# gnovack/distributed-training-and-deepspeed

Measured on AMD Instinct MI355X. Metric: tokens/sec (whole node) BERT-base DDP, higher is better.
Workload: dtype bf16; 1 GPU; model=bert-base-cased, params=108340804, global_batch=1024, per_gpu_batch=1024, seq_len=512, parallelism=dp1, grad_dtype=bfloat16, impl=fused, mlm_head=sparse (labelled rows only, static capacity 80896; identical loss/grads), optimizer=fused AdamW (transformers.AdamW hyper-params, lr 5e-5), tuned_gemms=True, hip_graph=False, force_collectives=False, prewarm=auto, async_wgrad=False, opt_overlap=True

## Files before the change

distributed_training_and_deepspeed_amd/ops/csrc/attention.hip:

```cpp
#include <stdio.h>
#include <type_traits>
#include <stdlib.h>
#include <string.h>

#include "common.h"

#ifndef DTD_ATTN_FUSED_BWD
#define DTD_ATTN_FUSED_BWD 0
#endif

using namespace dtd;

typedef float f32x16 __attribute__((ext_vector_type(16)));

namespace {

constexpr float kLog2e = 1.4426950408889634f;
constexpr float kLn2 = 0.6931471805599453f;

typedef short s16x4 __attribute__((ext_vector_type(4)));
typedef __attribute__((address_space(3))) s16x4 lds_s16x4;

__device__ __forceinline__ f32x16 mfma32(bf16x8 a, bf16x8 b, f32x16 c) {
  return __builtin_amdgcn_mfma_f32_32x32x16_bf16(a, b, c, 0, 0, 0);
// ... 396 lines not shown
    const bool slow = needmask || sl2 != 0.f;
    float tmax = -INFINITY;
    scores_kb(Knext, nxt, 0);
    if (slow) {
#pragma unroll
      for (int kb = 0; kb < NKB; ++kb)
#pragma unroll
        for (int i = 0; i < 16; ++i) {
          const int key = k0 + kb * 32 + crow(i, hh);
          float sv = fmaf(cur[kb][i], sc2, sl2 * (float)key);
          if (needmask && (key >= S || (a.causal && key > q))) sv = -INFINITY;
          cur[kb][i] = sv;
          tmax = fmaxf(tmax, sv);
        }
    } else {
#pragma unroll
      for (int kb = 0; kb < NKB; ++kb)
#pragma unroll
        for (int i = 0; i < 16; ++i) tmax = fmaxf(tmax, cur[kb][i]);
      tmax *= sc2;
    }
    tmax = xhalf_max(tmax);
    if (!__all(tmax - m <= a.thr)) {
      const float mnew = fmaxf(m, tmax);
      const float alpha = m == -INFINITY ? 0.f : fexp2(m - mnew);
      m = mnew;
      l *= alpha;
#pragma unroll
      for (int d = 0; d < NDB; ++d) oacc[d] *= alpha;
    }
    scores_kb(Knext, nxt, 1);
    const float mexp = m == -INFINITY ? 0.f : m;
    const float msc = slow ? 1.f : sc2;
    float ps[4];
#pragma unroll
    for (int kb = 0; kb < NKB; ++kb)
#pragma unroll
      for (int i = 0; i < 16; ++i) {
        const float pv = fexp2(fmaf(cur[kb][i], msc, -mexp));
        ps[i & 3] = (kb == 0 && i < 4) ? pv : ps[i & 3] + pv;
        cur[kb][i] = pv;
      }
    l += (ps[0] + ps[1]) + (ps[2] + ps[3]);
    if (drop) {
#pragma unroll
      for (int kb = 0; kb < NKB; ++kb) {
        const uint32_t mw = half_word(mwc[kb], hh);
#pragma unroll
        for (int i = 0; i < 16; ++i) cur[kb][i] = keep_bits(cur[kb][i], mw, crow(i, 0));
      }
    }
#pragma unroll
    for (int kb = 0; kb < NKB; ++kb)
#pragma unroll
      for (int s2 = 0; s2 < 2; ++s2) {
        bf16x8 pf;
#pragma unroll
        for (int j = 0; j < 8; ++j) pf[j] = (bf16)cur[kb][8 * s2 + j];
#pragma unroll
        for (int d = 0; d < NDB; ++d) oacc[d] = mfma32(tr_operand(V, VP, kb * 32 + 16 * s2, d * 32, lane), pf, oacc[d]);
      }
    if (t + 1 < nt) {
      if (t + 2 < nt) kl.store(Ks[t & 1], KP);
      vl.store(Vs[(t + 1) & 1], VP);
#pragma unroll
      for (int j = 0; j < NKB; ++j) mwc[j] = mwn[j];
      kl.load(ksrc, min(t + 3, last) * BN);
      vl.load(vsrc, min(t + 2, last) * BN);
      load_words(min(t + 2, last) * BN, mwn);
    }
    __syncthreads();
  };
  f32x16 sA[NKB], sB[NKB];
#pragma unroll
  for (int kb = 0; kb < NKB; ++kb) scores_kb(Ks[0], sA, kb);
  for (int t = 0; t < nt; t += 2) {
    tile_step(sA, sB, Ks[1], t);
    if (t + 1 < nt) tile_step(sB, sA, Ks[0], t + 1);
  }
  l = xhalf_sum(l);
  if (!qvalid) return;
  const float inv_l = l > 0.f ? inv_keep / l : 0.f;
  bf16* op = a.o + (size_t)(b * S + q) * a.ldo + h * D;
#pragma unroll
  for (int d = 0; d < NDB; ++d)
#pragma unroll
    for (int gq = 0; gq < 4; ++gq) {
      bf16x4 v4;
#pragma unroll
      for (int t = 0; t < 4; ++t) v4[t] = (bf16)(oacc[d][4 * gq + t] * inv_l);
      *reinterpret_cast<bf16x4*>(op + d * 32 + 8 * gq + 4 * hh) = v4;
    }
  if (hh == 0) a.lse[(size_t)bh * S + q] = (m + log2f(l)) * kLn2;
}

struct BwdArgs {
  const bf16* q; const bf16* k; const bf16* v; const bf16* dout; const float* lse; float* delta;
  const bf16* o;
  bf16* dq; bf16* dk; bf16* dv; const float* slopes;
  const uint32_t* maskA; const uint32_t* maskB;
  int B, S, H, ld, ldo, causal, W;
  float scale, p;
  float* bias_part;
  const int* kv_range;
  __device__ __forceinline__ int hkv() const { return W; }
  __device__ __forceinline__ int window() const { return __float_as_int(p); }
  __device__ __forceinline__ const int* doc() const { return kv_range; }
};

template <int S_>
__device__ __forceinline__ float xswz(float x) {
  return __int_as_float(__builtin_amdgcn_ds_swizzle(__float_as_int(x), (S_ << 10) | 0x1f));
}
template <int S_, int N>
__device__ __forceinline__ void rs_step(const float (&in)[2 * N], float (&out)[N], int r) {
  const bool hi = (r & S_) != 0;
#pragma unroll
  for (int j = 0; j < N; ++j) {
    const float mine = hi ? in[j + N] : in[j];
    const float other = hi ? in[j] : in[j + N];
    out[j] = mine + xswz<S_>(other);
  }
}
__device__ __forceinline__ float colsum32(const float (&v)[32], int r) {
  float a16[16], a8[8], a4[4], a2[2], a1[1];
  rs_step<16, 16>(v, a16, r);
  rs_step<8, 8>(a16, a8, r);
  rs_step<4, 4>(a8, a4, r);
  rs_step<2, 2>(a4, a2, r);
  rs_step<1, 1>(a2, a1, r);
  return a1[0];
}
__device__ __forceinline__ int colsum_col(int k, int hh) { return (k >> 4) * 32 + crow(k & 15, hh); }

template <int D, int OCC, int BM, bool DROP, bool ALIBI, bool MASK = true, bool RANGE = false>
__global__ void __launch_bounds__(256, OCC) attn_bwd_dkdv_kernel(BwdArgs a) {
  constexpr bool DOC = false, GQA = false, WIN = false;
#include "attention_bwd_dkdv_body.h"
}
template <int D, int OCC, int BM, bool DROP, bool ALIBI>
__global__ void __launch_bounds__(256, OCC) attn_bwd_dkdv_doc_kernel(BwdArgs a) {
  constexpr bool MASK = true, RANGE = false, DOC = true, GQA = false, WIN = false;
#include "attention_bwd_dkdv_body.h"
}
template <int D, int OCC, int BM, int MODE>
__global__ void __launch_bounds__(256, OCC) attn_bwd_dkdv_gqa_kernel(BwdArgs a) {
  constexpr bool DROP = false, ALIBI = false, MASK = true, RANGE = MODE == 1, DOC = MODE == 2, GQA = true, WIN = false;
#include "attention_bwd_dkdv_body.h"
}
template <int D, int OCC, int BM, int MODE>
__global__ void __launch_bounds__(256, OCC) attn_bwd_dkdv_win_kernel(BwdArgs a) {
  constexpr bool DROP = false, ALIBI = false, MASK = true, RANGE = MODE == 1, DOC = MODE == 2, GQA = true, WIN = true;
#include "attention_bwd_dkdv_body.h"
}

template <int D, int OCC, int BN, int RING, bool PK = false, bool RANGE = false>
__global__ void __launch_bounds__(256, OCC) attn_bwd_dq_kernel(BwdArgs a) {
  constexpr bool DOC = false, GQA = false, WIN = false;
#include "attention_bwd_dq_body.h"
}
template <int D, int OCC, int BN, int RING>
__global__ void __launch_bounds__(256, OCC) attn_bwd_dq_doc_kernel(BwdArgs a) {
  constexpr bool PK = false, RANGE = false, DOC = true, GQA = false, WIN = false;
#include "attention_bwd_dq_body.h"
}
template <int D, int OCC, int BN, int RING, int MODE>
__global__ void __launch_bounds__(256, OCC) attn_bwd_dq_gqa_kernel(BwdArgs a) {
  constexpr bool PK = false, RANGE = MODE == 1, DOC = MODE == 2, GQA = true, WIN = false;
#include "attention_bwd_dq_body.h"
}
template <int D, int OCC, int BN, int RING, int MODE>
__global__ void __launch_bounds__(256, OCC) attn_bwd_dq_win_kernel(BwdArgs a) {
  constexpr bool PK = false, RANGE = MODE == 1, DOC = MODE == 2, GQA = true, WIN = true;
#include "attention_bwd_dq_body.h"
}

#if DTD_ATTN_FUSED_BWD
__device__ __forceinline__ f32x4 mfma16(bf16x8 a, bf16x8 b, f32x4 c) {
  return __builtin_amdgcn_mfma_f32_16x16x32_bf16(a, b, c, 0, 0, 0);
}

__device__ __forceinline__ void mfma32_a(f32x16& acc, bf16x8 a, bf16x8 b) {
  asm volatile("s_nop 1\n\tv_mfma_f32_32x32x16_bf16 %0, %1, %2, %0" : "+a"(acc) : "v"(a), "v"(b));
}

__device__ __forceinline__ void mfma32_v0(f32x16& acc, bf16x8 a, bf16x8 b) {
  asm volatile("s_nop 1\n\tv_mfma_f32_32x32x16_bf16 %0, %1, %2, 0" : "=&v"(acc) : "v"(a), "v"(b));
}
__device__ __forceinline__ void mfma32_v(f32x16& acc, bf16x8 a, bf16x8 b) {
  asm volatile("s_nop 1\n\tv_mfma_f32_32x32x16_bf16 %0, %1, %2, %0" : "+v"(acc) : "v"(a), "v"(b));
}
__device__ __forceinline__ void mfma_vgpr_wait(f32x16& x, f32x16& y) {
  asm volatile("s_nop 11" : "+v"(x), "+v"(y));
}
__device__ __forceinline__ void mfma16_v(f32x4& acc, bf16x8 a, bf16x8 b) {
  asm volatile("s_nop 1\n\tv_mfma_f32_16x16x32_bf16 %0, %1, %2, %0" : "+v"(acc) : "v"(a), "v"(b));
}

template <int NKB, bool DROP>
__global__ void __launch_bounds__(256, 1) attn_bwd_fused_kernel(BwdArgs a) {
  constexpr int D = 64, NC = 4, NDB = 2, SK = 128 * NKB, KPW = 32 * NKB, NT = SK / 32;
  constexpr int KH = NKB % 2 == 0 ? 2 : 1, NH = NKB / KH;
  constexpr int DSP = 36;
  constexpr int DSR = 4 * KH * 32;
  struct Smem {
    float lse_s[32], del_s[32];
    bf16 Qs[32 * 64];
    bf16 Os[32 * 64];
    bf16 DS[DSR * DSP];
    bf16 Ks[SK * 64];
    bf16 Vs[SK * 64];
  };
  __shared__ __attribute__((aligned(16))) Smem sm;

  const int tid = threadIdx.x, lane = tid & 63, w = __builtin_amdgcn_readfirstlane(tid >> 6), hh = lane >> 5,
            r = lane & 31;
  const int bh = blockIdx.x, b = bh / a.H, h = bh % a.H;
  const int S = a.S;
  const float sc2 = a.scale * kLog2e;
  const float inv_keep = DROP ? 1.f / (1.f - a.p) : 1.f;
  const int kw0 = w * KPW;
  const int Sp = 32 * a.W;
  const float* lseb = a.lse + (size_t)bh * S;
  const RowSrc qsrc = row_src<D>(a.q + (size_t)b * S * a.ld + h * D, a.ld, S);
  const RowSrc dsrc = row_src<D>(a.dout + (size_t)b * S * a.ldo + h * D, a.ldo, S);
  const RowSrc osrc = row_src<D>(a.o + (size_t)b * S * a.ldo + h * D, a.ldo, S);
  {
    const RowSrc ksrc = row_src<D>(a.k + (size_t)b * S * a.ld + h * D, a.ld, S);
    const RowSrc vsrc = row_src<D>(a.v + (size_t)b * S * a.ld + h * D, a.ld, S);
#pragma unroll
    for (int half = 0; half < 2; ++half) {
      TileLoader<D, SK / 2> kl, vl;
      kl.load(ksrc, half * (SK / 2));
      vl.load(vsrc, half * (SK / 2));
      kl.store_swz(sm.Ks + half * (SK / 2) * 64);
      vl.store_swz(sm.Vs + half * (SK / 2) * 64);
    }
  }
  TileLoader<D, 32> ql, dl, ol;
  float lse_n = 0.f;
  auto fetch = [&](int q0) {
    ql.load(qsrc, q0);
    dl.load(dsrc, q0);
    ol.load(osrc, q0);
    if (tid < 32) lse_n = lseb[q0 + tid];
  };
  auto stage = [&]() {
    float part = 0.f;
#pragma unroll
    for (int j = 0; j < 8; ++j) part = fmaf((float)dl.reg[0][j], (float)ol.reg[0][j], part);
    part += __shfl_xor(part, 1, 64);
    part += __shfl_xor(part, 2, 64);
    part += __shfl_xor(part, 4, 64);
    ql.store_swz(sm.Qs);
    dl.store_swz(sm.Os);
    if ((tid & 7) == 0) sm.del_s[tid >> 3] = -part;
    if (tid < 32) sm.lse_s[tid] = -lse_n * kLog2e;
  };
  fetch(0);
  stage();

  f32x16 dk[NKB][NDB], dv[NKB][NDB];
#pragma unroll
  for (int kb = 0; kb < NKB; ++kb)
#pragma unroll
    for (int d = 0; d < NDB; ++d) { dk[kb][d] = f32x16{}; dv[kb][d] = f32x16{}; }
  const int g16 = lane >> 4, l16 = lane & 15, qq = l16 >> 2, pp = l16 & 3;
  const int kcol = 16 * w + 4 * pp;
  __syncthreads();

  for (int t = 0; t < NT; ++t) {
    const int q0 = t * 32;
    if (t + 1 < NT) fetch(q0 + 32);
    f32x4 dq2[2] = {f32x4{}, f32x4{}};
#pragma unroll
    for (int hf = 0; hf < NH; ++hf) {
#pragma unroll
      for (int kk = 0; kk < KH; ++kk) {
        const int kb = hf * KH + kk;
        const int key0 = kw0 + 32 * kb;
        f32x16 sacc, pacc;
#pragma unroll
        for (int c = 0; c < NC; ++c) {
          const bf16x8 qa = swz_row_read(sm.Qs, 0, r, 2 * c + hh), kr = swz_row_read(sm.Ks, key0, r, 2 * c + hh);
          const bf16x8 oa = swz_row_read(sm.Os, 0, r, 2 * c + hh), vr = swz_row_read(sm.Vs, key0, r, 2 * c + hh);
          if (c == 0) { mfma32_v0(sacc, qa, kr); mfma32_v0(pacc, oa, vr); }
          else { mfma32_v(sacc, qa, kr); mfma32_v(pacc, oa, vr); }
        }
        mfma_vgpr_wait(sacc, pacc);
        uint64_t mk[16];
        if constexpr (DROP) {
          const cu64* mp = (const cu64*)(uintptr_t)(a.maskA + ((size_t)bh * a.W + min(w * NKB + kb, a.W - 1)) * Sp +
                                                    keep_off(q0, Sp));
#pragma unroll
          for (int i = 0; i < 16; ++i) mk[i] = mp[i];
        }
        f32x4 L4[4];
#pragma unroll
        for (int g = 0; g < 4; ++g) L4[g] = *reinterpret_cast<const f32x4*>(&sm.lse_s[8 * g + 4 * hh]);
        const f32x2 sc2v = pk2(sc2, sc2);
#pragma unroll
        for (int i = 0; i < 16; i += 2) {
          const f32x2 x = pk_fma(pk2(sacc[i], sacc[i + 1]), sc2v, pk2(L4[i >> 2][i & 3], L4[i >> 2][(i & 3) + 1]));
          sacc[i] = fexp2(x.x);
          sacc[i + 1] = fexp2(x.y);
        }
// ... 229 lines not shown
      for (int g = 0; g < 4; ++g) L4[g] = *reinterpret_cast<const f32x4*>(&sm.lse_s[8 * g + 4 * hh]);
      const f32x2 sc2v = pk2(sc2, sc2);
#pragma unroll
      for (int i = 0; i < 16; i += 2) {
        const f32x2 x = pk_fma(pk2(sacc[i], sacc[i + 1]), sc2v, pk2(L4[i >> 2][i & 3], L4[i >> 2][(i & 3) + 1]));
        sacc[i] = fexp2(x.x);
        sacc[i + 1] = fexp2(x.y);
      }
      f32x4 D4[4];
#pragma unroll
      for (int g = 0; g < 4; ++g) D4[g] = *reinterpret_cast<const f32x4*>(&sm.del_s[8 * g + 4 * hh]);
#pragma unroll
      for (int i = 0; i < 16; i += 2) {
        const f32x2 nd = pk2(D4[i >> 2][i & 3], D4[i >> 2][(i & 3) + 1]);
        if constexpr (DROP) {
          const f32x2 tt = pk_fma(pk2(sel_keep(pacc[i], mk[i]), sel_keep(pacc[i + 1], mk[i + 1])),
                                  pk2(inv_keep, inv_keep), nd);
          const f32x2 ds = pk2(sacc[i], sacc[i + 1]) * tt;
          pacc[i] = ds.x;
          pacc[i + 1] = ds.y;
          sacc[i] = sel_keep(sacc[i], mk[i]);
          sacc[i + 1] = sel_keep(sacc[i + 1], mk[i + 1]);
        } else {
          const f32x2 ds = pk2(sacc[i], sacc[i + 1]) * (pk2(pacc[i], pacc[i + 1]) + nd);
          pacc[i] = ds.x;
          pacc[i + 1] = ds.y;
        }
      }
      bf16* dsrow = sm.DS + (w * 32 + r) * DSP + 4 * hh;
#pragma unroll
      for (int s2 = 0; s2 < 2; ++s2) {
        bf16x8 pb, sb;
#pragma unroll
        for (int j = 0; j < 8; ++j) { pb[j] = (bf16)sacc[8 * s2 + j]; sb[j] = (bf16)pacc[8 * s2 + j]; }
#pragma unroll
        for (int d = 0; d < NDB; ++d) {
          dv[kb][d] = mfma32(tr_operand_swz(sm.Os, 16 * s2, d * 32, lane), pb, dv[kb][d]);
          dk[kb][d] = mfma32(tr_operand_swz(sm.Qs, 16 * s2, d * 32, lane), sb, dk[kb][d]);
        }
        *reinterpret_cast<bf16x4*>(dsrow + 16 * s2) = __builtin_shufflevector(sb, sb, 0, 1, 2, 3);
        *reinterpret_cast<bf16x4*>(dsrow + 16 * s2 + 8) = __builtin_shufflevector(sb, sb, 4, 5, 6, 7);
      }
      __syncthreads();
#pragma unroll 1
      for (int k0 = 0; k0 < DSR; k0 += 32) {
        const int key = (k0 / 32) * KPW + kb * 32 + 8 * g16 + qq;
        const bf16* ka = sm.Ks + key * 64 + 8 * ((kcol >> 3) ^ swz64(key)) + (kcol & 7);
        const bf16* kb4 = sm.Ks + (key + 4) * 64 + 8 * ((kcol >> 3) ^ swz64(key + 4)) + (kcol & 7);
        const int lr = k0 + 8 * g16 + qq;
        const bf16* dp = sm.DS + lr * DSP + 16 * qh + 4 * pp;
        dq1 = mfma16(cat(tr_read(ka), tr_read(kb4)), cat(tr_read(dp), tr_read(dp + 4 * DSP)), dq1);
      }
      float cs[4] = {0.f, 0.f, 0.f, 0.f};
      if (kb == NH - 1) {
        bf16x4 v4;
#pragma unroll
        for (int j = 0; j < 4; ++j) {
          v4[j] = (bf16)(dq1[j] * a.scale);
          cs[j] = (float)v4[j];
        }
        *reinterpret_cast<bf16x4*>(a.dq + (size_t)(b * S + q0 + 16 * qh + l16) * a.ld + h * D + 16 * dd + 4 * g16) = v4;
        if (a.bias_part) {
#pragma unroll
          for (int j = 0; j < 4; ++j) {
            cs[j] += __shfl_xor(cs[j], 1, 64);
            cs[j] += __shfl_xor(cs[j], 2, 64);
            cs[j] += __shfl_xor(cs[j], 4, 64);
            cs[j] += __shfl_xor(cs[j], 8, 64);
          }
          if (qh == 1 && l16 == 0)
            *reinterpret_cast<f32x4*>(&sm.csq[16 * dd + 4 * g16]) = f32x4{cs[0], cs[1], cs[2], cs[3]};
        }
        if (t + 1 < NT) stage();
      }
      __syncthreads();
      if (kb == NH - 1 && a.bias_part && qh == 0 && l16 == 0) {
        const f32x4 o4 = *reinterpret_cast<const f32x4*>(&sm.csq[16 * dd + 4 * g16]);
        *reinterpret_cast<f32x4*>(a.bias_part + ((size_t)b * (S / 32) + t) * (3 * a.H * D) + h * D + 16 * dd + 4 * g16) =
            f32x4{cs[0] + o4[0], cs[1] + o4[1], cs[2] + o4[2], cs[3] + o4[3]};
      }
    }
  }
  const float dv_scale = inv_keep;
  auto put = [&](const f32x16 (&acc)[NDB], float sc, bf16* dst, int colbase, int kb) {
    if (a.bias_part) {
      float vk[32];
#pragma unroll
      for (int d = 0; d < NDB; ++d)
#pragma unroll
        for (int i = 0; i < 16; ++i) vk[16 * d + i] = (float)(bf16)(acc[d][i] * sc);
      const float sk = colsum32(vk, r);
      a.bias_part[((size_t)b * (S / 32) + w * NKBW + kb) * (3 * a.H * D) + colbase + h * D + colsum_col(r, hh)] = sk;
    }
    bf16* p = dst + (size_t)(b * S + kw0 + 32 * kb + r) * a.ld + h * D;
#pragma unroll
    for (int d = 0; d < NDB; ++d)
#pragma unroll
      for (int gq = 0; gq < 4; ++gq) {
        bf16x4 k4;
#pragma unroll
        for (int j = 0; j < 4; ++j) k4[j] = (bf16)(acc[d][4 * gq + j] * sc);
        *reinterpret_cast<bf16x4*>(p + d * 32 + 8 * gq + 4 * hh) = k4;
      }
  };
#pragma unroll
  for (int kb = 0; kb < NKBW; ++kb) {
    put(dk[kb], a.scale, a.dk, a.H * D, kb);
    __builtin_amdgcn_sched_barrier(0);
    put(dv[kb], dv_scale, a.dv, 2 * a.H * D, kb);
    __builtin_amdgcn_sched_barrier(0);
  }
}

#endif

}

static int occupancy(int which) {
  static const int defaults[3] = {3, 2, 3};
  const char* env = getenv("DTD_ATTN_OCC");
  if (!env) return defaults[which];
  int v[3] = {defaults[0], defaults[1], defaults[2]};
  sscanf(env, "%d,%d,%d", &v[0], &v[1], &v[2]);
  return v[which];
}

static bool fwd_pipe() {
  const char* e = getenv("DTD_ATTN_FWD");
  return e != nullptr && strcmp(e, "pipe") == 0;
}

static bool fwd_pk() {
  const char* e = getenv("DTD_ATTN_FWD_PK");
  return e != nullptr && e[0] == '1';
}

static int tile_keys(int which) {
  static const int defaults[2] = {64, 64};
  const char* env = getenv("DTD_ATTN_TILE");
  if (!env) return defaults[which];
  int v[2] = {defaults[0], defaults[1]};
  sscanf(env, "%d,%d", &v[0], &v[1]);
  return v[which];
}

static int g_bwd_form = -1;
static int bwd_form() {
  if (g_bwd_form < 0) {
    const char* e = getenv("DTD_ATTN_BWD");
    g_bwd_form = !e ? 0 : strcmp(e, "fused") == 0 ? 1 : strcmp(e, "fused4") == 0 ? 2 : 0;
  }
  return g_bwd_form;
}
static bool bwd_fused() { return bwd_form() != 0; }
static bool bwd_fused8() { return bwd_form() == 1; }


enum Family { kMha = 0, kGqa = 1, kWin = 2 };

static int mode_of(const int* kv_range, const int* doc) { return doc ? 2 : kv_range ? 1 : 0; }

template <int N, class F>
static void with_const(int v, F&& f) {
  if (v >= N - 1) return f(std::integral_constant<int, N - 1>{});
  if constexpr (N > 1) with_const<N - 1>(v, f);
}
template <class F>
static void with_family(Family fam, F&& f) {
  if (fam == kMha) f(std::integral_constant<int, kMha>{});
  else if (fam == kGqa) f(std::integral_constant<int, kGqa>{});
  else f(std::integral_constant<int, kWin>{});
}

static bool offsets_fit(int S, int ld, int ldo) {
  const long long lim = 0x7fffffffLL;
  const long long W = (S + 31) / 32;
  return (long long)S * ld * 2 < lim && (long long)S * ldo * 2 < lim && 32 * W * W * 4 < lim;
}

static int check_call(Family fam, int B, int S, int H, int Hkv, int D, int ld, int ldo, int causal, int window,
                      const int* kv_range, const int* doc) {
  if (B * S * H == 0) return -1;
  if (fam == kWin && (window <= 0 || !causal)) return (int)hipErrorInvalidValue;
  if (fam != kMha && (Hkv <= 0 || Hkv > H || H % Hkv || (fam == kGqa && Hkv == H))) return (int)hipErrorInvalidValue;
  if (kv_range && doc) return (int)hipErrorInvalidValue;
  if (D != 64 && D != 128) return (int)hipErrorInvalidValue;
  if (!offsets_fit(S, ld, ldo)) return (int)hipErrorInvalidValue;
  return 0;
}

static float rescale_thr() {
  const char* e = getenv("DTD_ATTN_RESCALE_THR");
  return e ? (float)atof(e) : kRescaleThr;
}

static float window_bits(int window) {
  float f;
  memcpy(&f, &window, sizeof f);
  return f;
}

static FwdArgs fwd_args(const void* q, const void* k, const void* v, void* o, float* lse, const float* slopes,
                        const uint32_t* masks, int B, int S, int H, int ld, int ldo, int causal, float scale, float p,
                        int hkv, int window, const int* kv_range, const int* doc) {
  const int W = (S + 31) / 32;
  FwdArgs a{(const bf16*)q, (const bf16*)k, (const bf16*)v, (bf16*)o, lse, slopes, masks,
            masks ? masks + (size_t)B * H * (32 * W) * W : nullptr, B, S, H, ld, ldo, causal, hkv ? hkv : W,
            scale, p, rescale_thr(), doc ? doc : kv_range};
  if (window) a.causal = 1, a.p = window_bits(window < S ? window : S);
  return a;
}
static BwdArgs bwd_args(const void* q, const void* k, const void* v, const void* o, const void* dout, const float* lse,
                        float* delta, const uint32_t* masks, void* dq, void* dk, void* dv, const float* slopes, int B,
                        int S, int H, int ld, int ldo, int causal, float scale, float p, float* bias_part, int hkv,
                        int window, const int* kv_range, const int* doc) {
  const int W = (S + 31) / 32;
  BwdArgs a{(const bf16*)q, (const bf16*)k, (const bf16*)v, (const bf16*)dout, lse, delta, (const bf16*)o,
            (bf16*)dq, (bf16*)dk, (bf16*)dv, slopes, masks, masks ? masks + (size_t)B * H * (32 * W) * W : nullptr,
            B, S, H, ld, ldo, causal, hkv ? hkv : W, scale, p, bias_part, doc ? doc : kv_range};
  if (window) a.causal = 1, a.p = window_bits(window < S ? window : S);
  return a;
}

template <int D> struct TileForm;
template <> struct TileForm<64> { static constexpr int OCC = 3, BN = 64, RING = 1, KV_OCC = 2, KV_BM = 128; };
template <> struct TileForm<128> { static constexpr int OCC = 1, BN = 64, RING = 2, KV_OCC = 1, KV_BM = 64; };

static void launch_masks(uint32_t* masks, int B, int S, int H, float p, const uint64_t* rng, uint32_t sid, hipStream_t s) {
  const int W = (S + 31) / 32;
  hipLaunchKernelGGL(attn_mask_kernel, dim3((S + 255) / 256, B * H), dim3(256), 0, s, masks,
                     masks + (size_t)B * H * (32 * W) * W, S, W, rng, sid, keep_threshold(p));
}

template <int D>
static void launch_fwd_plain(dim3 grid, hipStream_t s, const FwdArgs& a) {
  if constexpr (D == 128) {
    hipLaunchKernelGGL((attn_fwd_kernel<128, 1, 64, 2>), grid, dim3(256), 0, s, a);
  } else if (fwd_pipe()) {
    hipLaunchKernelGGL((attn_fwd_pipe_kernel<64, 2, 64>), grid, dim3(256), 0, s, a);
  } else {
    const int o = occupancy(0);
    if (o >= 3 && fwd_pk()) hipLaunchKernelGGL((attn_fwd_kernel<64, 3, 64, 1, true>), grid, dim3(256), 0, s, a);
    else if (o >= 3) hipLaunchKernelGGL((attn_fwd_kernel<64, 3, 64, 1>), grid, dim3(256), 0, s, a);
    else if (o == 2) hipLaunchKernelGGL((attn_fwd_kernel<64, 2, 64, 2>), grid, dim3(256), 0, s, a);
    else hipLaunchKernelGGL((attn_fwd_kernel<64, 1, 64, 2>), grid, dim3(256), 0, s, a);
  }
}

template <int D, int FAM, int MODE>
static void launch_fwd_form(dim3 grid, hipStream_t s, const FwdArgs& a) {
  using T = TileForm<D>;
  if constexpr (FAM == kWin) hipLaunchKernelGGL((attn_fwd_win_kernel<D, T::OCC, T::BN, T::RING, MODE>), grid, dim3(256), 0, s, a);
  else if constexpr (FAM == kGqa) hipLaunchKernelGGL((attn_fwd_gqa_kernel<D, T::OCC, T::BN, T::RING, MODE>), grid, dim3(256), 0, s, a);
  else if constexpr (MODE == 2) hipLaunchKernelGGL((attn_fwd_doc_kernel<D, T::OCC, T::BN, T::RING>), grid, dim3(256), 0, s, a);
  else if constexpr (MODE == 1) hipLaunchKernelGGL((attn_fwd_kernel<D, T::OCC, T::BN, T::RING, false, true>), grid, dim3(256), 0, s, a);
  else launch_fwd_plain<D>(grid, s, a);
}

static int attn_fwd_launch(Family fam, const void* q, const void* k, const void* v, void* o, float* lse,
                           const float* slopes, uint32_t* masks, int B, int S, int H, int Hkv, int D, int ld, int ldo,
                           int causal, float scale, float p, const uint64_t* rng, uint32_t sid, int window,
                           const int* kv_range, const int* doc, hipStream_t s) {
  if (const int rc = check_call(fam, B, S, H, Hkv, D, ld, ldo, causal, window, kv_range, doc)) return rc < 0 ? 0 : rc;
  if (p > 0.f && !masks) return (int)hipErrorInvalidValue;
  if (p > 0.f && rng) launch_masks(masks, B, S, H, p, rng, sid, s);
  const FwdArgs a = fwd_args(q, k, v, o, lse, slopes, p > 0.f ? masks : nullptr, B, S, H, ld, ldo, causal, scale, p,
                             fam == kMha ? 0 : Hkv, window, kv_range, doc);
  const dim3 grid((S + 127) / 128, B * H);
  with_family(fam, [&](auto f) { with_const<3>(mode_of(kv_range, doc), [&](auto m) {
    constexpr int FAM = decltype(f)::value, MODE = decltype(m)::value;
    if (D == 64) launch_fwd_form<64, FAM, MODE>(grid, s, a);
    else launch_fwd_form<128, FAM, MODE>(grid, s, a);
  }); });
  DTD_LAUNCH_CHECK();
}

DTD_EXPORT int dtd_attn_fwd(const void* q, const void* k, const void* v, void* o, float* lse, const float* slopes,
                            uint32_t* masks, int B, int S, int H, int D, int ld, int ldo, int causal, float scale,
                            float p, const uint64_t* rng, uint32_t sid, hipStream_t s) {
  return attn_fwd_launch(kMha, q, k, v, o, lse, slopes, masks, B, S, H, H, D, ld, ldo, causal, scale, p, rng, sid, 0,
                         nullptr, nullptr, s);
}

DTD_EXPORT int dtd_attn_fwd_range(const void* q, const void* k, const void* v, void* o, float* lse,
                                  const float* slopes, uint32_t* masks, int B, int S, int H, int D, int ld, int ldo,
                                  int causal, float scale, float p, const uint64_t* rng, uint32_t sid,
                                  const int* kv_range, hipStream_t s) {
  if (!kv_range) return (int)hipErrorInvalidValue;
  return attn_fwd_launch(kMha, q, k, v, o, lse, slopes, masks, B, S, H, H, D, ld, ldo, causal, scale, p, rng, sid, 0,
                         kv_range, nullptr, s);
}

DTD_EXPORT int dtd_attn_fwd_doc(const void* q, const void* k, const void* v, void* o, float* lse, const float* slopes,
                                uint32_t* masks, int B, int S, int H, int D, int ld, int ldo, int causal, float scale,
                                float p, const uint64_t* rng, uint32_t sid, const int* doc, hipStream_t s) {
  if (!doc) return (int)hipErrorInvalidValue;
  return attn_fwd_launch(kMha, q, k, v, o, lse, slopes, masks, B, S, H, H, D, ld, ldo, causal, scale, p, rng, sid, 0,
                         nullptr, doc, s);
}

DTD_EXPORT int dtd_attn_fwd_gqa(const void* q, const void* k, const void* v, void* o, float* lse, int B, int S, int H,
                                int Hkv, int D, int ld, int ldo, int causal, float scale, const int* kv_range,
                                const int* doc, hipStream_t s) {
  return attn_fwd_launch(kGqa, q, k, v, o, lse, nullptr, nullptr, B, S, H, Hkv, D, ld, ldo, causal, scale, 0.f, nullptr,
                         0, 0, kv_range, doc, s);
}

DTD_EXPORT int dtd_attn_fwd_win(const void* q, const void* k, const void* v, void* o, float* lse, int B, int S, int H,
                                int Hkv, int D, int ld, int ldo, int causal, float scale, int window,
                                const int* kv_range, const int* doc, hipStream_t s) {
  return attn_fwd_launch(kWin, q, k, v, o, lse, nullptr, nullptr, B, S, H, Hkv, D, ld, ldo, causal, scale, 0.f, nullptr,
                         0, window, kv_range, doc, s);
}

DTD_EXPORT int dtd_attn_fused_bwd_built() { return DTD_ATTN_FUSED_BWD; }

DTD_EXPORT int dtd_attn_set_bwd_form(int f) {
  const int old = bwd_form();
  g_bwd_form = f < 0 || f > 2 ? 0 : f;
  return old;
}

DTD_EXPORT int dtd_attn_masks(uint32_t* masks, int B, int S, int H, float p, const uint64_t* rng, uint32_t sid,
                              hipStream_t s) {
  if (B * S * H == 0 || p <= 0.f) return 0;
  if (!masks || !rng) return (int)hipErrorInvalidValue;
  launch_masks(masks, B, S, H, p, rng, sid, s);
  DTD_LAUNCH_CHECK();
}

template <int D, int OCC, int BM>
static void launch_dkdv(dim3 grid, hipStream_t s, const BwdArgs& a) {
  const bool drop = a.maskB != nullptr, alibi = a.slopes != nullptr;
  if (!a.causal && a.S % 128 == 0 && !alibi) {
    if (drop) hipLaunchKernelGGL((attn_bwd_dkdv_kernel<D, OCC, BM, true, false, false>), grid, dim3(256), 0, s, a);
    else hipLaunchKernelGGL((attn_bwd_dkdv_kernel<D, OCC, BM, false, false, false>), grid, dim3(256), 0, s, a);
    return;
  }
  if (drop && alibi) hipLaunchKernelGGL((attn_bwd_dkdv_kernel<D, OCC, BM, true, true>), grid, dim3(256), 0, s, a);
  else if (drop) hipLaunchKernelGGL((attn_bwd_dkdv_kernel<D, OCC, BM, true, false>), grid, dim3(256), 0, s, a);
  else if (alibi) hipLaunchKernelGGL((attn_bwd_dkdv_kernel<D, OCC, BM, false, true>), grid, dim3(256), 0, s, a);
  else hipLaunchKernelGGL((attn_bwd_dkdv_kernel<D, OCC, BM, false, false>), grid, dim3(256), 0, s, a);
}

template <int D, int OCC, int BM, int MODE>
static void launch_dkdv_masked(dim3 grid, hipStream_t s, const BwdArgs& a) {
  with_const<2>(a.maskB != nullptr, [&](auto drop) { with_const<2>(a.slopes != nullptr, [&](auto alibi) {
    constexpr bool DROP = decltype(drop)::value, ALIBI = decltype(alibi)::value;
    if constexpr (MODE == 2) hipLaunchKernelGGL((attn_bwd_dkdv_doc_kernel<D, OCC, BM, DROP, ALIBI>), grid, dim3(256), 0, s, a);
    else hipLaunchKernelGGL((attn_bwd_dkdv_kernel<D, OCC, BM, DROP, ALIBI, true, true>), grid, dim3(256), 0, s, a);
  }); });
}

static int g_bwd_kernels = 3;
DTD_EXPORT int dtd_attn_set_bwd_kernels(int mask) {
  const int old = g_bwd_kernels;
  g_bwd_kernels = mask & 3;
  return old;
}

template <int D>
static void launch_bwd_plain(dim3 grid, bool run_dq, bool run_dkdv, hipStream_t s, const BwdArgs& a) {
#if DTD_ATTN_FUSED_BWD
  if (D == 64 && !a.causal && !a.slopes && a.S % 128 == 0 && a.S <= 512 && bwd_fused()) {
    const bool drop = a.maskA != nullptr;
    const dim3 g1(a.B * a.H);
    if (a.S == 512 && bwd_fused8()) {
      if (drop) hipLaunchKernelGGL((attn_bwd_fused8_kernel<2, true>), g1, dim3(512), 0, s, a);
      else hipLaunchKernelGGL((attn_bwd_fused8_kernel<2, false>), g1, dim3(512), 0, s, a);
      return;
    }
    switch (a.S / 128) {
      case 1: if (drop) hipLaunchKernelGGL((attn_bwd_fused_kernel<1, true>), g1, dim3(256), 0, s, a);
              else hipLaunchKernelGGL((attn_bwd_fused_kernel<1, false>), g1, dim3(256), 0, s, a); break;
      case 2: if (drop) hipLaunchKernelGGL((attn_bwd_fused_kernel<2, true>), g1, dim3(256), 0, s, a);
              else hipLaunchKernelGGL((attn_bwd_fused_kernel<2, false>), g1, dim3(256), 0, s, a); break;
      case 3: if (drop) hipLaunchKernelGGL((attn_bwd_fused_kernel<3, true>), g1, dim3(256), 0, s, a);
              else hipLaunchKernelGGL((attn_bwd_fused_kernel<3, false>), g1, dim3(256), 0, s, a); break;
      default: if (drop) hipLaunchKernelGGL((attn_bwd_fused_kernel<4, true>), g1, dim3(256), 0, s, a);
               else hipLaunchKernelGGL((attn_bwd_fused_kernel<4, false>), g1, dim3(256), 0, s, a); break;
    }
    return;
  }
#endif
  if constexpr (D == 64) {
    const int o = occupancy(2);
    if (!run_dq) {}
    else if (tile_keys(1) == 128) hipLaunchKernelGGL((attn_bwd_dq_kernel<64, 2, 128, 2>), grid, dim3(256), 0, s, a);
    else if (o >= 3 && fwd_pk()) hipLaunchKernelGGL((attn_bwd_dq_kernel<64, 3, 64, 1, true>), grid, dim3(256), 0, s, a);
    else if (o >= 3) hipLaunchKernelGGL((attn_bwd_dq_kernel<64, 3, 64, 1>), grid, dim3(256), 0, s, a);
    else if (o == 2) hipLaunchKernelGGL((attn_bwd_dq_kernel<64, 2, 64, 2>), grid, dim3(256), 0, s, a);
    else hipLaunchKernelGGL((attn_bwd_dq_kernel<64, 1, 64, 2>), grid, dim3(256), 0, s, a);
    const int bm = getenv("DTD_ATTN_DKDV_BM") ? atoi(getenv("DTD_ATTN_DKDV_BM")) : 128;
    if (!run_dkdv) {}
    else if (bm == 128 && occupancy(1) == 1) launch_dkdv<64, 1, 128>(grid, s, a);
    else if (bm == 128) launch_dkdv<64, 2, 128>(grid, s, a);
    else if (occupancy(1) >= 2) launch_dkdv<64, 2, 64>(grid, s, a);
    else launch_dkdv<64, 1, 64>(grid, s, a);
  } else {
    if (run_dq) hipLaunchKernelGGL((attn_bwd_dq_kernel<128, 1, 64, 2>), grid, dim3(256), 0, s, a);
    if (run_dkdv) launch_dkdv<128, 1, 64>(grid, s, a);
  }
}

template <int D, int FAM, int MODE>
static void launch_bwd_form(dim3 gq, dim3 gkv, bool run_dq, bool run_dkdv, hipStream_t s, const BwdArgs& a) {
  using T = TileForm<D>;
  if constexpr (FAM == kMha && MODE == 0) return launch_bwd_plain<D>(gq, run_dq, run_dkdv, s, a);
  if (run_dq) {
    if constexpr (FAM == kWin) hipLaunchKernelGGL((attn_bwd_dq_win_kernel<D, T::OCC, T::BN, T::RING, MODE>), gq, dim3(256), 0, s, a);
    else if constexpr (FAM == kGqa) hipLaunchKernelGGL((attn_bwd_dq_gqa_kernel<D, T::OCC, T::BN, T::RING, MODE>), gq, dim3(256), 0, s, a);
    else if constexpr (MODE == 2) hipLaunchKernelGGL((attn_bwd_dq_doc_kernel<D, T::OCC, T::BN, T::RING>), gq, dim3(256), 0, s, a);
    else hipLaunchKernelGGL((attn_bwd_dq_kernel<D, T::OCC, T::BN, T::RING, false, true>), gq, dim3(256), 0, s, a);
  }
  if (run_dkdv) {
    if constexpr (FAM == kWin) hipLaunchKernelGGL((attn_bwd_dkdv_win_kernel<D, T::KV_OCC, T::KV_BM, MODE>), gkv, dim3(256), 0, s, a);
    else if constexpr (FAM == kGqa) hipLaunchKernelGGL((attn_bwd_dkdv_gqa_kernel<D, T::KV_OCC, T::KV_BM, MODE>), gkv, dim3(256), 0, s, a);
    else launch_dkdv_masked<D, T::KV_OCC, T::KV_BM, MODE>(gkv, s, a);
  }
}

static int attn_bwd_launch(Family fam, const void* q, const void* k, const void* v, const void* o, const void* dout,
                           const float* lse, float* delta, const uint32_t* masks, void* dq, void* dk, void* dv,
                           const float* slopes, int B, int S, int H, int Hkv, int D, int ld, int ldo, int causal,
                           float scale, float p, float* bias_part, int window, const int* kv_range, const int* doc,
                           hipStream_t s) {
  if (const int rc = check_call(fam, B, S, H, Hkv, D, ld, ldo, causal, window, kv_range, doc)) return rc < 0 ? 0 : rc;
  if (p > 0.f && !masks) return (int)hipErrorInvalidValue;
  const BwdArgs a = bwd_args(q, k, v, o, dout, lse, delta, p > 0.f ? masks : nullptr, dq, dk, dv, slopes, B, S, H, ld, ldo,
                             causal, scale, p, D == 64 ? bias_part : nullptr, fam == kMha ? 0 : Hkv, window, kv_range, doc);
  const dim3 gq((S + 127) / 128, B * H), gkv((S + 127) / 128, B * Hkv);
  const bool run_dq = g_bwd_kernels & 1, run_dkdv = g_bwd_kernels & 2;
  with_family(fam, [&](auto f) { with_const<3>(mode_of(kv_range, doc), [&](auto m) {
    constexpr int FAM = decltype(f)::value, MODE = decltype(m)::value;
    if (D == 64) launch_bwd_form<64, FAM, MODE>(gq, gkv, run_dq, run_dkdv, s, a);
    else launch_bwd_form<128, FAM, MODE>(gq, gkv, run_dq, run_dkdv, s, a);
  }); });
  DTD_LAUNCH_CHECK();
}

DTD_EXPORT int dtd_attn_bwd(const void* q, const void* k, const void* v, const void* o, const void* dout,
                            const float* lse, float* delta, const uint32_t* masks, void* dq, void* dk, void* dv,
                            const float* slopes, int B, int S, int H, int D, int ld, int ldo, int causal, float scale,
                            float p, float* bias_part, hipStream_t s) {
  return attn_bwd_launch(kMha, q, k, v, o, dout, lse, delta, masks, dq, dk, dv, slopes, B, S, H, H, D, ld, ldo, causal,
                         scale, p, bias_part, 0, nullptr, nullptr, s);
}

DTD_EXPORT int dtd_attn_bwd_range(const void* q, const void* k, const void* v, const void* o, const void* dout,
                                  const float* lse, float* delta, const uint32_t* masks, void* dq, void* dk, void* dv,
                                  const float* slopes, int B, int S, int H, int D, int ld, int ldo, int causal,
                                  float scale, float p, float* bias_part, const int* kv_range, hipStream_t s) {
  if (!kv_range) return (int)hipErrorInvalidValue;
  return attn_bwd_launch(kMha, q, k, v, o, dout, lse, delta, masks, dq, dk, dv, slopes, B, S, H, H, D, ld, ldo, causal,
                         scale, p, bias_part, 0, kv_range, nullptr, s);
}

DTD_EXPORT int dtd_attn_bwd_doc(const void* q, const void* k, const void* v, const void* o, const void* dout,
                                const float* lse, float* delta, const uint32_t* masks, void* dq, void* dk, void* dv,
                                const float* slopes, int B, int S, int H, int D, int ld, int ldo, int causal,
                                float scale, float p, float* bias_part, const int* doc, hipStream_t s) {
  if (!doc) return (int)hipErrorInvalidValue;
  return attn_bwd_launch(kMha, q, k, v, o, dout, lse, delta, masks, dq, dk, dv, slopes, B, S, H, H, D, ld, ldo, causal,
                         scale, p, bias_part, 0, nullptr, doc, s);
}

DTD_EXPORT int dtd_attn_bwd_gqa(const void* q, const void* k, const void* v, const void* o, const void* dout,
                                const float* lse, float* delta, void* dq, void* dk, void* dv, int B, int S, int H,
                                int Hkv, int D, int ld, int ldo, int causal, float scale, const int* kv_range,
                                const int* doc, hipStream_t s) {
  return attn_bwd_launch(kGqa, q, k, v, o, dout, lse, delta, nullptr, dq, dk, dv, nullptr, B, S, H, Hkv, D, ld, ldo,
                         causal, scale, 0.f, nullptr, 0, kv_range, doc, s);
}

DTD_EXPORT int dtd_attn_bwd_win(const void* q, const void* k, const void* v, const void* o, const void* dout,
                                const float* lse, float* delta, void* dq, void* dk, void* dv, int B, int S, int H,
                                int Hkv, int D, int ld, int ldo, int causal, float scale, int window,
                                const int* kv_range, const int* doc, hipStream_t s) {
  return attn_bwd_launch(kWin, q, k, v, o, dout, lse, delta, nullptr, dq, dk, dv, nullptr, B, S, H, Hkv, D, ld, ldo,
                         causal, scale, 0.f, nullptr, window, kv_range, doc, s);
}
```

Before: 1.495 million tokens/s.

## Add double-buffered DMA-pipelined dK/dV attention backward kernel for D=64

Adds a specialized dK/dV backward kernel for head dim 64 with 128-row query tiles. It double-buffers Q and dO tiles in LDS via direct buffer-to-LDS DMA, prefetches LSE, delta and dropout mask words for the next tile, and software-pipelines the score MFMAs of the next 32-row block against the softmax and gradient MFMAs of the current one. This is meant to hide global-memory latency and raise MFMA utilization in the attention backward pass. It becomes the default for non-causal, non-ALiBi cases with S divisible by 128. The cost is a new code path with manual waitcnt and scheduling barriers, higher register pressure, and a fixed occupancy of 2.

```diff
diff --git a/distributed_training_and_deepspeed_amd/ops/csrc/attention.hip b/distributed_training_and_deepspeed_amd/ops/csrc/attention.hip
--- a/distributed_training_and_deepspeed_amd/ops/csrc/attention.hip
+++ b/distributed_training_and_deepspeed_amd/ops/csrc/attention.hip
@@ -572,6 +572,11 @@
 __global__ void __launch_bounds__(256, OCC) attn_bwd_dkdv_win_kernel(BwdArgs a) {
   constexpr bool DROP = false, ALIBI = false, MASK = true, RANGE = MODE == 1, DOC = MODE == 2, GQA = true, WIN = true;
 #include "attention_bwd_dkdv_body.h"
+}
+template <int N> __device__ __forceinline__ void wait_vm() { asm volatile("s_waitcnt vmcnt(%0)" :: "n"(N) : "memory"); }
+template <bool DROP, bool PIPE>
+__global__ void __launch_bounds__(256, 2) attn_bwd_dkdv_pipe_kernel(BwdArgs a) {
+#include "attention_bwd_dkdv_pipe_body.h"
 }
 
 template <int D, int OCC, int BN, int RING, bool PK = false, bool RANGE = false>
@@ -1107,6 +1112,11 @@
   }
   return g_bwd_form;
 }
+constexpr int kDkdvFormDefault = 2;
+static int dkdv_form() {
+  const char* e = getenv("DTD_ATTN_DKDV");
+  return !e ? kDkdvFormDefault : strcmp(e, "old") == 0 ? 0 : strcmp(e, "dma") == 0 ? 1 : strcmp(e, "pipe") == 0 ? 2 : kDkdvFormDefault;
+}
 static bool bwd_fused() { return bwd_form() != 0; }
 static bool bwd_fused8() { return bwd_form() == 1; }
 
@@ -1348,6 +1358,12 @@
     else hipLaunchKernelGGL((attn_bwd_dq_kernel<64, 1, 64, 2>), grid, dim3(256), 0, s, a);
     const int bm = getenv("DTD_ATTN_DKDV_BM") ? atoi(getenv("DTD_ATTN_DKDV_BM")) : 128;
     if (!run_dkdv) {}
+    else if (bm == 128 && occupancy(1) != 1 && !a.causal && !a.slopes && a.S % 128 == 0 && dkdv_form() != 0) {
+      with_const<2>(a.maskB != nullptr, [&](auto drop) { with_const<2>(dkdv_form() == 2, [&](auto pipe) {
+        constexpr bool DROP = decltype(drop)::value, PIPE = decltype(pipe)::value;
+        hipLaunchKernelGGL((attn_bwd_dkdv_pipe_kernel<DROP, PIPE>), grid, dim3(256), 0, s, a);
+      }); });
+    }
     else if (bm == 128 && occupancy(1) == 1) launch_dkdv<64, 1, 128>(grid, s, a);
     else if (bm == 128) launch_dkdv<64, 2, 128>(grid, s, a);
     else if (occupancy(1) >= 2) launch_dkdv<64, 2, 64>(grid, s, a);
diff --git a/distributed_training_and_deepspeed_amd/ops/csrc/attention_bwd_dkdv_pipe_body.h b/distributed_training_and_deepspeed_amd/ops/csrc/attention_bwd_dkdv_pipe_body.h
--- /dev/null
+++ b/distributed_training_and_deepspeed_amd/ops/csrc/attention_bwd_dkdv_pipe_body.h
@@ -0,0 +1,225 @@
+  constexpr int D = 64, BM = 128, NC = D / 16, NDB = D / 32;
+  struct Smem {
+    float lse_s[2][BM], del_s[2][BM];
+    bf16 Qs[2][BM * D];
+    bf16 Os[2][BM * D];
+  };
+  __shared__ __attribute__((aligned(16))) Smem sm;
+  auto& lse_s = sm.lse_s;
+  auto& del_s = sm.del_s;
+  auto& Qs = sm.Qs;
+  auto& Os = sm.Os;
+
+  const int lane = threadIdx.x & 63, w = __builtin_amdgcn_readfirstlane(threadIdx.x >> 6), hh = lane >> 5,
+            r = lane & 31;
+  int tx, ty;
+  xcd_tile(tx, ty);
+  const int bh = ty, b = bh / a.H, h = bh % a.H;
+  const int S = a.S;
+  const int kblk = tx * 128;
+  const int key = kblk + w * 32 + r;
+  const float sc2 = a.scale * kLog2e;
+  const float inv_keep = DROP ? 1.f / (1.f - a.p) : 1.f;
+  const int Sp = 32 * a.W;
+  const uint32_t* mrow = DROP ? a.maskA + ((size_t)bh * a.W + min((kblk >> 5) + w, a.W - 1)) * Sp : nullptr;
+  const __amdgpu_buffer_rsrc_t mrs = bounded_rsrc(DROP ? (const void*)mrow : (const void*)a.lse, DROP ? (uint32_t)Sp * 4u : 0u);
+  const __amdgpu_buffer_rsrc_t q_rs = bounded_rsrc(a.q + (size_t)b * S * a.ld + h * D, (uint32_t)(((S - 1) * a.ld + D) * 2));
+  const __amdgpu_buffer_rsrc_t o_rs = bounded_rsrc(a.dout + (size_t)b * S * a.ldo + h * D, (uint32_t)(((S - 1) * a.ldo + D) * 2));
+  const __amdgpu_buffer_rsrc_t lse_rs = bounded_rsrc(a.lse + (size_t)bh * S, (uint32_t)S * 4u);
+  const __amdgpu_buffer_rsrc_t del_rs = bounded_rsrc(a.delta + (size_t)bh * S, (uint32_t)S * 4u);
+
+  bf16x8 kf[NC], vf[NC];
+  load_frags<D>(kf, a.k + (size_t)b * S * a.ld + h * D, a.ld, S, key, hh);
+  load_frags<D>(vf, a.v + (size_t)b * S * a.ld + h * D, a.ld, S, key, hh);
+  f32x16 dk[NDB], dv[NDB];
+#pragma unroll
+  for (int d = 0; d < NDB; ++d) { dk[d] = f32x16{}; dv[d] = f32x16{}; }
+
+  const int nt = S / BM;
+  const int dma_row = lane >> 3, dma_ch = ((lane & 7) ^ swz64(8 * (w & 1) + dma_row)) * 8;
+  const int q_voff = (dma_row * a.ld + dma_ch) * 2, o_voff = (dma_row * a.ldo + dma_ch) * 2;
+  const int q_ld2 = a.ld * 2, o_ld2 = a.ldo * 2;
+  auto dma_tile = [&](int nb, int q0) {
+    const uint32_t ql = lds_addr(Qs[nb]), ol = lds_addr(Os[nb]);
+#pragma unroll
+    for (int i = 0; i < BM / 32; ++i) dma16(q_rs, ql + (32 * i + 8 * w) * (D * 2), q_voff, (q0 + 32 * i + 8 * w) * q_ld2);
+#pragma unroll
+    for (int i = 0; i < BM / 32; ++i) dma16(o_rs, ol + (32 * i + 8 * w) * (D * 2), o_voff, (q0 + 32 * i + 8 * w) * o_ld2);
+  };
+  float lse_r = 0.f, del_r = 0.f;
+  const int stat_off = threadIdx.x < BM ? (int)threadIdx.x * 4 : 0x40000000;
+  auto load_stats = [&](int q0) {
+    lse_r = load_stat(lse_rs, q0 * 4 + stat_off);
+    del_r = load_stat(del_rs, q0 * 4 + stat_off);
+  };
+  auto store_stats = [&](int buf) {
+    if (threadIdx.x < BM) {
+      lse_s[buf][threadIdx.x] = -lse_r * kLog2e;
+      del_s[buf][threadIdx.x] = -del_r * (DROP ? 1.f - a.p : 1.f);
+    }
+  };
+  constexpr int NPF = BM / 64;
+  uint32_t pfw[NPF] = {};
+  auto prefetch_words = [&](int q0) {
+#pragma unroll
+    for (int j = 0; j < NPF; ++j) {
+      asm volatile("" :: "v"(pfw[j]));
+      pfw[j] = __builtin_amdgcn_raw_buffer_load_b32(mrs, (lane + 64 * j) * 4, q0 * 4, 0);
+    }
+  };
+  auto row_reads = [&](const bf16* Q, const bf16* O, int qb, bf16x8 (&qa)[NC], bf16x8 (&oa)[NC]) {
+#pragma unroll
+    for (int c = 0; c < NC; ++c) {
+      qa[c] = swz_row_read(Q, qb * 32, r, 2 * c + hh);
+      oa[c] = swz_row_read(O, qb * 32, r, 2 * c + hh);
+    }
+  };
+  auto score_mfmas = [&](const bf16x8 (&qa)[NC], const bf16x8 (&oa)[NC], f32x16& sacc, f32x16& pacc) {
+    sacc = f32x16{};
+    pacc = f32x16{};
+#pragma unroll
+    for (int c = 0; c < NC; ++c) {
+      sacc = mfma32(qa[c], kf[c], sacc);
+      pacc = mfma32(oa[c], vf[c], pacc);
+    }
+  };
+  auto scores = [&](const bf16* Q, const bf16* O, int qb, f32x16& sacc, f32x16& pacc) {
+    bf16x8 qa[NC], oa[NC];
+    row_reads(Q, O, qb, qa, oa);
+    score_mfmas(qa, oa, sacc, pacc);
+  };
+  auto load_keep = [&](int qrow0, uint64_t (&mk)[16]) {
+    if constexpr (DROP) {
+      const cu64* mp = (const cu64*)(uintptr_t)(mrow + keep_off(qrow0, Sp));
+#pragma unroll
+      for (int i = 0; i < 16; ++i) mk[i] = mp[i];
+    }
+  };
+  auto read_stats = [&](int buf, int qb, f32x4 (&L4)[4], f32x4 (&D4)[4]) {
+#pragma unroll
+    for (int g = 0; g < 4; ++g) {
+      L4[g] = *reinterpret_cast<const f32x4*>(&lse_s[buf][qb * 32 + 8 * g + 4 * hh]);
+      D4[g] = *reinterpret_cast<const f32x4*>(&del_s[buf][qb * 32 + 8 * g + 4 * hh]);
+    }
+  };
+  auto softmax = [&](f32x16& sacc, f32x16& pacc, const uint64_t (&mk)[16], const f32x4 (&L4)[4], const f32x4 (&D4)[4]) {
+    const f32x2 sc2v = pk2(sc2, sc2);
+#pragma unroll
+    for (int i = 0; i < 16; i += 2) {
+      const f32x2 nl = pk2(L4[i >> 2][i & 3], L4[i >> 2][(i & 3) + 1]);
+      const f32x2 x = pk_fma(pk2(sacc[i], sacc[i + 1]), sc2v, nl);
+      sacc[i] = fexp2(x.x);
+      sacc[i + 1] = fexp2(x.y);
+    }
+#pragma unroll
+    for (int i = 0; i < 16; i += 2) {
+      const f32x2 nd = pk2(D4[i >> 2][i & 3], D4[i >> 2][(i & 3) + 1]);
+      if constexpr (DROP) {
+        const f32x2 pm = pk2(sel_keep(sacc[i], mk[i]), sel_keep(sacc[i + 1], mk[i + 1]));
+        const f32x2 u = pk2(sacc[i], sacc[i + 1]) * nd;
+        const f32x2 ds = pk_fma(pm, pk2(pacc[i], pacc[i + 1]), u);
+        pacc[i] = ds.x;
+        pacc[i + 1] = ds.y;
+        sacc[i] = pm.x;
+        sacc[i + 1] = pm.y;
+      } else {
+        const f32x2 ds = pk2(sacc[i], sacc[i + 1]) * (pk2(pacc[i], pacc[i + 1]) + nd);
+        pacc[i] = ds.x;
+        pacc[i + 1] = ds.y;
+      }
+    }
+  };
+  auto grads = [&](const bf16* Q, const bf16* O, int qb, const f32x16& sacc, const f32x16& pacc) {
+#pragma unroll
+    for (int s = 0; s < 2; ++s) {
+      bf16x8 pb, sb;
+#pragma unroll
+      for (int j = 0; j < 8; ++j) { pb[j] = (bf16)sacc[8 * s + j]; sb[j] = (bf16)pacc[8 * s + j]; }
+#pragma unroll
+      for (int d = 0; d < NDB; ++d) {
+        dv[d] = mfma32(tr_operand_swz(O, qb * 32 + 16 * s, d * 32, lane), pb, dv[d]);
+        dk[d] = mfma32(tr_operand_swz(Q, qb * 32 + 16 * s, d * 32, lane), sb, dk[d]);
+      }
+    }
+  };
+
+  load_stats(0);
+  dma_tile(0, 0);
+  store_stats(0);
+#pragma unroll
+  for (int c = 0; c < NC; ++c) asm volatile("" : "+v"(kf[c]), "+v"(vf[c]));
+  wait_vm<0>();
+  __syncthreads();
+  for (int t = 0; t < nt; ++t) {
+    const int buf = t & 1, q0 = t * BM;
+    if (t + 1 < nt) {
+      load_stats(q0 + BM);
+      if (DROP) prefetch_words(q0 + BM);
+      dma_tile(buf ^ 1, q0 + BM);
+    }
+    const bf16* Q = Qs[buf];
+    const bf16* O = Os[buf];
+    if constexpr (PIPE) {
+      f32x16 sacc[2], pacc[2];
+      scores(Q, O, 0, sacc[0], pacc[0]);
+#pragma unroll
+      for (int qb = 0; qb < BM / 32; ++qb) {
+        const int cur = qb & 1;
+        __builtin_amdgcn_sched_barrier(0);
+        uint64_t mk[16];
+        f32x4 L4[4], D4[4];
+        read_stats(buf, qb, L4, D4);
+        if constexpr (DROP) {
+          bf16x8 qa[NC], oa[NC];
+          if (qb + 1 < BM / 32) {
+            row_reads(Q, O, qb + 1, qa, oa);
+#pragma unroll
+            for (int c = 0; c < NC; ++c) asm volatile("" : "+v"(qa[c]), "+v"(oa[c]));
+          }
+#pragma unroll
+          for (int g = 0; g < 4; ++g) asm volatile("" : "+v"(L4[g]), "+v"(D4[g]));
+          __builtin_amdgcn_sched_barrier(0);
+          load_keep(q0 + qb * 32, mk);
+          if (qb + 1 < BM / 32) score_mfmas(qa, oa, sacc[cur ^ 1], pacc[cur ^ 1]);
+        } else {
+          if (qb + 1 < BM / 32) scores(Q, O, qb + 1, sacc[cur ^ 1], pacc[cur ^ 1]);
+        }
+        __builtin_amdgcn_sched_barrier(0);
+        softmax(sacc[cur], pacc[cur], mk, L4, D4);
+        grads(Q, O, qb, sacc[cur], pacc[cur]);
+      }
+    } else {
+#pragma unroll 1
+      for (int qb = 0; qb < BM / 32; ++qb) {
+        f32x16 sacc, pacc;
+        uint64_t mk[16];
+        f32x4 L4[4], D4[4];
+        scores(Q, O, qb, sacc, pacc);
+        load_keep(q0 + qb * 32, mk);
+        read_stats(buf, qb, L4, D4);
+        softmax(sacc, pacc, mk, L4, D4);
+        grads(Q, O, qb, sacc, pacc);
+      }
+    }
+    if (t + 1 < nt) store_stats(buf ^ 1);
+    wait_vm<0>();
+    __syncthreads();
+  }
+  const float dv_scale = inv_keep;
+  const float dk_scale = a.scale * inv_keep;
+  if (a.bias_part) {
+    float vk[32], vv[32];
+#pragma unroll
+    for (int d = 0; d < NDB; ++d)
+#pragma unroll
+      for (int i = 0; i < 16; ++i) {
+        vk[16 * d + i] = (float)(bf16)(dk[d][i] * dk_scale);
+        vv[16 * d + i] = (float)(bf16)(dv[d][i] * dv_scale);
+      }
+    const float sk = colsum32(vk, r), sv = colsum32(vv, r);
+    float* row = a.bias_part + ((size_t)b * gridDim.x * 4 + (kblk >> 5) + w) * (3 * a.H * D) + h * D + colsum_col(r, hh);
+    row[a.H * D] = sk;
+    row[2 * a.H * D] = sv;
+  }
+  store_rows16<NDB>(a.dk + (size_t)(b * S + key) * a.ld + h * D, dk, dk_scale, hh, true);
+  store_rows16<NDB>(a.dv + (size_t)(b * S + key) * a.ld + h * D, dv, dv_scale, hh, true);
```

After: 1.511 million tokens/s, median of 6. 1.01x the previous value.
